# pkzhou/PointSLOT

Hardware: AMD Instinct MI355X
Metric: tracked frames/sec KITTI stereo 1242x375 (higher is better)
Workload: dtype u8

## Files before the change

### pointslot_amd/csrc/orb_plan.h

```cpp
#pragma once
#include <stdint.h>

#define PS_ORB_MAX_LEVELS 8
#define PS_EDGE 19
#define PS_MINB 16
#define PS_QT_NCAP 2048
#define PS_FAST_WIN 66

struct OrbLevel {
  int32_t w, h;
  int32_t stride;
  int32_t bstride;
  uint32_t plane_off;
  uint32_t blur_off;
  int32_t n_cols, n_rows;
  int32_t w_cell, h_cell;
  int32_t cell_base;
  int32_t cell_cap;
  uint32_t cand_off;
  uint32_t key_off;
  int32_t key_cap;
  int32_t quota;
  int32_t n_ini;
  float h_x;
  int32_t sel_off;
  int32_t sel_cap;
  float scale;
  float inv_scale;
  float kp_size;
  uint32_t xtab_off, ytab_off;
  int32_t blur_blk_base;
  int32_t border_blk_base;
};

struct OrbPlan {
  OrbLevel lv[PS_ORB_MAX_LEVELS];
  int32_t nlevels;
  int32_t img_w, img_h;
  int32_t n_cells;
  int32_t sel_total;
  int32_t kp_cap;
  int32_t ini_th, min_th;
  int32_t blur_blocks;
  int32_t border_blocks;
  uint64_t arena_bytes;
  uint64_t cellcnt_off;
  uint64_t cand_base;
  uint64_t key_base;
  uint64_t sel_base;
  uint64_t selcnt_off;
  uint64_t ncand_off;
  uint32_t celltab_off;
};

struct StPair {
  const uint8_t* arena_l; const uint8_t* arena_r;
  const void* kps_l; const uint8_t* desc_l; const int32_t* cnt_l;
  const void* kps_r; const uint8_t* desc_r; const int32_t* cnt_r;
  float* u_right; float* depth; int32_t* sad; int32_t* kept;
  uint8_t* scratch;
};
#define PS_ST_MAXB 512
#define PS_ST_CAP 4096
#define PS_ST_OFF_BYTES ((PS_ST_MAXB + 4) * 4)
#define PS_ST_SCRATCH (PS_ST_OFF_BYTES + PS_ST_CAP * 4 + PS_ST_CAP * 8)
```

### pointslot_amd/csrc/orb_stereo.hip

```cpp
#include <hip/hip_runtime.h>
#include <stdint.h>
#include "orb_plan.h"

namespace {

#define ST_G(T) const __attribute__((address_space(1))) T
#define ST_GM(T) __attribute__((address_space(1))) T
template <typename T> __device__ __forceinline__ ST_G(T)* st_g(const T* p) { return (ST_G(T)*)p; }
template <typename T> __device__ __forceinline__ ST_GM(T)* st_gm(T* p) { return (ST_GM(T)*)p; }

typedef uint32_t st_u4 __attribute__((ext_vector_type(4)));
typedef uint32_t st_u2 __attribute__((ext_vector_type(2)));
struct PsKeyPoint { float x, y, size, angle, response; int32_t octave, class_id; };

__device__ __forceinline__ int hamming256(const st_u4 a0, const st_u4 a1, const st_u4 b0, const st_u4 b1) {
  return __popc(a0.x ^ b0.x) + __popc(a0.y ^ b0.y) + __popc(a0.z ^ b0.z) + __popc(a0.w ^ b0.w) +
         __popc(a1.x ^ b1.x) + __popc(a1.y ^ b1.y) + __popc(a1.z ^ b1.z) + __popc(a1.w ^ b1.w);
}
__device__ __forceinline__ uint32_t wave_min_u32(uint32_t v) {
  v = min(v, (uint32_t)__builtin_amdgcn_update_dpp((int)v, (int)v, 0xB1, 0xF, 0xF, false));
  v = min(v, (uint32_t)__builtin_amdgcn_update_dpp((int)v, (int)v, 0x4E, 0xF, 0xF, false));
  v = min(v, (uint32_t)__builtin_amdgcn_update_dpp((int)v, (int)v, 0x141, 0xF, 0xF, false));
  v = min(v, (uint32_t)__builtin_amdgcn_update_dpp((int)v, (int)v, 0x140, 0xF, 0xF, false));
  const uint32_t a = (uint32_t)__builtin_amdgcn_readlane((int)v, 0), b = (uint32_t)__builtin_amdgcn_readlane((int)v, 16);
  const uint32_t c = (uint32_t)__builtin_amdgcn_readlane((int)v, 32), d = (uint32_t)__builtin_amdgcn_readlane((int)v, 48);
  return min(min(a, b), min(c, d));
}
__device__ __forceinline__ int wave_sum_i32(int v) {
  v += __builtin_amdgcn_update_dpp(0, v, 0xB1, 0xF, 0xF, true);
  v += __builtin_amdgcn_update_dpp(0, v, 0x4E, 0xF, 0xF, true);
  v += __builtin_amdgcn_update_dpp(0, v, 0x141, 0xF, 0xF, true);
  v += __builtin_amdgcn_update_dpp(0, v, 0x140, 0xF, 0xF, true);
  return __builtin_amdgcn_readlane(v, 0) + __builtin_amdgcn_readlane(v, 16) + __builtin_amdgcn_readlane(v, 32) + __builtin_amdgcn_readlane(v, 48);
}

__global__ __launch_bounds__(256) void st_bucket(OrbPlan plan, const StPair* pairs) {
  __shared__ int cnt[PS_ST_MAXB + 1], fill[PS_ST_MAXB];
  const StPair S = pairs[blockIdx.x];
  const int Nr = min(*S.cnt_r, PS_ST_CAP), tid = threadIdx.x;
  const PsKeyPoint* KR = reinterpret_cast<const PsKeyPoint*>(S.kps_r);
  int32_t* boff = reinterpret_cast<int32_t*>(S.scratch);
  int32_t* bidx = reinterpret_cast<int32_t*>(S.scratch + PS_ST_OFF_BYTES);
  uint2* rinfo = reinterpret_cast<uint2*>(S.scratch + PS_ST_OFF_BYTES + PS_ST_CAP * 4);
  const int nb = min(PS_ST_MAXB, (plan.img_h >> 3) + 1);
  for (int b = tid; b <= PS_ST_MAXB; b += 256) { cnt[b] = 0; if (b < PS_ST_MAXB) fill[b] = 0; }
  __syncthreads();
  for (int iR = tid; iR < Nr; iR += 256) {
    const PsKeyPoint kr = KR[iR];
    const float r = __fmul_rn(2.0f, plan.lv[kr.octave].scale);
    const int maxr = (int)ceilf(__fadd_rn(kr.y, r)), minr = (int)floorf(__fsub_rn(kr.y, r));
    (void)maxr; (void)minr;
    atomicAdd(&cnt[min(max((int)kr.y >> 3, 0), nb - 1)], 1);
  }
  __syncthreads();
  if (tid == 0) { int acc = 0; for (int b = 0; b <= nb; b++) { const int c = cnt[b]; cnt[b] = acc; acc += c; } }
  __syncthreads();
  for (int b = tid; b <= nb; b += 256) boff[b] = cnt[b];
  for (int iR = tid; iR < Nr; iR += 256) {
    const PsKeyPoint kr = KR[iR];
    const int b = min(max((int)kr.y >> 3, 0), nb - 1);
    const int pos = cnt[b] + atomicAdd(&fill[b], 1);
    const float r = __fmul_rn(2.0f, plan.lv[kr.octave].scale);
    const int maxr = (int)ceilf(__fadd_rn(kr.y, r)), minr = (int)floorf(__fsub_rn(kr.y, r));
    bidx[pos] = iR;
    rinfo[pos] = make_uint2(__float_as_uint(kr.x), (uint32_t)(min(max(minr + 1024, 0), 8191)) | ((uint32_t)(min(max(maxr + 1024, 0), 8191)) << 13) | ((uint32_t)kr.octave << 26));
  }
}

typedef unsigned short st_us2 __attribute__((ext_vector_type(2)));
__device__ __forceinline__ uint32_t row_min_u32(uint32_t v) {
  v = min(v, (uint32_t)__builtin_amdgcn_update_dpp((int)v, (int)v, 0xB1, 0xF, 0xF, false));
  v = min(v, (uint32_t)__builtin_amdgcn_update_dpp((int)v, (int)v, 0x4E, 0xF, 0xF, false));
  v = min(v, (uint32_t)__builtin_amdgcn_update_dpp((int)v, (int)v, 0x141, 0xF, 0xF, false));
  v = min(v, (uint32_t)__builtin_amdgcn_update_dpp((int)v, (int)v, 0x140, 0xF, 0xF, false));
  return v;
}
__device__ __forceinline__ int row_sum_i32(int v) {
  v += __builtin_amdgcn_update_dpp(0, v, 0xB1, 0xF, 0xF, true);
  v += __builtin_amdgcn_update_dpp(0, v, 0x4E, 0xF, 0xF, true);
  v += __builtin_amdgcn_update_dpp(0, v, 0x141, 0xF, 0xF, true);
  v += __builtin_amdgcn_update_dpp(0, v, 0x140, 0xF, 0xF, true);
  return v;
}
#define ST_PAIR(hi, lo, b0, b1) __builtin_amdgcn_perm(hi, lo, (uint32_t)(b0) | 0x0c000c00u | ((uint32_t)(b1) << 16))

__global__ __launch_bounds__(256) void st_match(OrbPlan plan, const StPair* pairs, float mb, float mbf, int npairs) {
  __shared__ float s_scale[PS_ORB_MAX_LEVELS], s_inv[PS_ORB_MAX_LEVELS];
  __shared__ int s_w[PS_ORB_MAX_LEVELS], s_stride[PS_ORB_MAX_LEVELS];
  __shared__ uint32_t s_plane[PS_ORB_MAX_LEVELS];
#pragma unroll
  for (int l = 0; l < PS_ORB_MAX_LEVELS; l++)
    if ((int)threadIdx.x == l) { s_scale[l] = plan.lv[l].scale; s_inv[l] = plan.lv[l].inv_scale; s_w[l] = plan.lv[l].w; s_stride[l] = plan.lv[l].stride; s_plane[l] = plan.lv[l].plane_off; }
  __syncthreads();
  const int pair = (int)blockIdx.y * 8 + ((int)blockIdx.x & 7);
  if (pair >= npairs) return;
  const StPair S = pairs[pair];
  const int wave = __builtin_amdgcn_readfirstlane(threadIdx.x >> 6), lane = threadIdx.x & 63, grp = lane >> 4, l16 = lane & 15;
  const int N = *st_g(S.cnt_l);
  const int iL0 = ((int)blockIdx.x >> 3) * 16 + wave * 4;
  if (iL0 >= N) return;
  const int iL = iL0 + grp;
  const bool live = iL < N;
  ST_G(PsKeyPoint)* KL = st_g(reinterpret_cast<const PsKeyPoint*>(S.kps_l));
  const int iLc = live ? iL : N - 1;
  PsKeyPoint kpL;
  kpL.x = KL[iLc].x; kpL.y = KL[iLc].y; kpL.octave = KL[iLc].octave;
  float out_ur = -1.0f, out_depth = -1.0f;
  int out_sad = -1;
  const float minD = 0.f, maxD = __fdiv_rn(mbf, mb);
  const float uL = kpL.x, vL = kpL.y;
  const int levelL = kpL.octave;
  const int rowL = (int)vL;
  const float minU = __fsub_rn(uL, maxD), maxU = __fsub_rn(uL, minD);
  uint32_t best = 0xFFFFFFFFu;
  float best_rx = 0.f;
  if (live && !(maxU < 0)) {
    ST_G(st_u4)* dl = st_g(reinterpret_cast<const st_u4*>(S.desc_l + (size_t)iL * 32));
    const st_u4 a0 = dl[0], a1 = dl[1];
    ST_G(int32_t)* boff = st_g(reinterpret_cast<const int32_t*>(S.scratch));
    ST_G(int32_t)* bidx = st_g(reinterpret_cast<const int32_t*>(S.scratch + PS_ST_OFF_BYTES));
    ST_G(st_u2)* rinfo = st_g(reinterpret_cast<const st_u2*>(S.scratch + PS_ST_OFF_BYTES + PS_ST_CAP * 4));
    const int nb = min(PS_ST_MAXB, (plan.img_h >> 3) + 1);
    const float rmax = __fadd_rn(__fmul_rn(2.0f, plan.lv[plan.nlevels - 1].scale), 2.0f);
    const int b0 = min(max((int)floorf((float)rowL - rmax) >> 3, 0), nb - 1), b1 = min(max((int)ceilf((float)rowL + rmax) >> 3, 0), nb - 1);
    const int k_end = boff[b1 + 1];
    const uint32_t rowk = (uint32_t)(rowL + 1024);
    for (int k = boff[b0] + l16; k < k_end; k += 64) {
      st_u2 ri[4]; int iR[4];
#pragma unroll
      for (int u = 0; u < 4; u++) { const int ku = min(k + 16 * u, k_end - 1); ri[u] = rinfo[ku]; iR[u] = bidx[ku]; }
#pragma unroll
      for (int u = 0; u < 4; u++) {
        if (k + 16 * u >= k_end) continue;
        const uint32_t minr = ri[u].y & 0x1FFF, maxr = (ri[u].y >> 13) & 0x1FFF;
        const int oct = (int)(ri[u].y >> 26);
        if (rowk < minr || rowk > maxr) continue;
        if ((uint32_t)(oct - levelL + 1) > 2u) continue;
        const float rx = __uint_as_float(ri[u].x);
        if (!(rx >= minU && rx <= maxU)) continue;
        ST_G(st_u4)* dr = st_g(reinterpret_cast<const st_u4*>(S.desc_r + (size_t)iR[u] * 32));
        const uint32_t d = (uint32_t)hamming256(a0, a1, dr[0], dr[1]);
        if (d < 100u) {
          const uint32_t key = (d << 16) | (uint32_t)iR[u];
          if (key < best) { best = key; best_rx = rx; }
        }
      }
    }
  }
  const uint32_t lane_best = best;
  best = row_min_u32(best);
  float uR0 = 0.f;
  {
    const uint32_t owners = (uint32_t)(__ballot(lane_best == best && best != 0xFFFFFFFFu) >> (lane & 48)) & 0xFFFFu;
    uR0 = __shfl(best_rx, (lane & 48) + (owners ? __ffs((int)owners) - 1 : 0));
  }
  const int bestDist = best == 0xFFFFFFFFu ? 100 : (int)(best >> 16);
  if (bestDist < 75) {
    const float Lscale = s_scale[levelL], Linv = s_inv[levelL];
    const int Lw = s_w[levelL], Lstride = s_stride[levelL];
    const uint32_t Lplane = s_plane[levelL];
    const float scaleduL = roundf(__fmul_rn(kpL.x, Linv));
    const float scaledvL = roundf(__fmul_rn(kpL.y, Linv));
    const float scaleduR0 = roundf(__fmul_rn(uR0, Linv));
    const float iniu = scaleduR0 + 5 - 5, endu = scaleduR0 + 5 + 5 + 1;
    if (!(iniu < 0 || endu >= (float)Lw)) {
      const int cy = (int)scaledvL, cxl = (int)scaleduL, cxr = (int)scaleduR0;
      const int i = min(l16, 10);
      ST_G(uint8_t)* al = st_g(S.arena_l);
      ST_G(uint8_t)* ar = st_g(S.arena_r);
      ST_G(uint32_t)* pl = (ST_G(uint32_t)*)(al + (Lplane + (uint32_t)((PS_EDGE + cy + i - 5) * Lstride + PS_EDGE + cxl - 5)));
      ST_G(uint32_t)* pr = (ST_G(uint32_t)*)(ar + (Lplane + (uint32_t)((PS_EDGE + cy + i - 5) * Lstride + PS_EDGE + cxr - 10)));
      ST_G(uint32_t)* prc = (ST_G(uint32_t)*)(ar + (Lplane + (uint32_t)((PS_EDGE + cy) * Lstride + PS_EDGE + cxr - 10)));
      uint32_t lw[3], rw[6], cw[6];
#pragma unroll
      for (int q = 0; q < 3; q++) lw[q] = pl[q];
#pragma unroll
      for (int q = 0; q < 6; q++) { rw[q] = pr[q]; cw[q] = prc[q]; }
      const uint32_t Lc = al[Lplane + (uint32_t)((PS_EDGE + cy) * Lstride + PS_EDGE + cxl)];
      const uint32_t biasA = (256u - Lc) * 0x00010001u;
      uint32_t a[6];
#pragma unroll
      for (int q = 0; q < 5; q++) a[q] = ST_PAIR(lw[q >> 1], lw[q >> 1], (2 * q) & 3, (2 * q + 1) & 3) + biasA;
      a[5] = ST_PAIR(0u, lw[2], 2, 0x0c) + (biasA & 0xFFFFu);
      uint32_t E[11], O[10];
#pragma unroll
      for (int q = 0; q < 11; q++) {
        const int b0i = 2 * q, b1i = 2 * q + 1;
        E[q] = ST_PAIR(rw[b0i >> 2], rw[b0i >> 2], b0i & 3, q == 10 ? 0x0c : (b1i & 3));
      }
#pragma unroll
      for (int q = 0; q < 10; q++) {
        const int b0i = 2 * q + 1, b1i = 2 * q + 2;
        O[q] = ST_PAIR(rw[b1i >> 2], rw[b0i >> 2], b0i & 3, (b1i & 3) + ((b1i >> 2) != (b0i >> 2) ? 4 : 0));
      }
      int dists[11];
#pragma unroll
      for (int s = 0; s < 11; s++) {
        const uint32_t Rc = (cw[(s + 5) >> 2] >> (8 * ((s + 5) & 3))) & 0xFFu;
        const uint32_t biasB = (256u - Rc) * 0x00010001u;
        uint32_t acc = 0;
#pragma unroll
        for (int q = 0; q < 5; q++) {
          const uint32_t r2 = (s & 1) ? O[(s - 1) / 2 + q] : E[s / 2 + q];
          acc = __builtin_amdgcn_sad_u16(a[q], r2 + biasB, acc);
        }
        const uint32_t rl = ((s & 1) ? O[(s - 1) / 2 + 5] : E[s / 2 + 5]) & 0xFFFFu;
        acc = __builtin_amdgcn_sad_u16(a[5], rl + (biasB & 0xFFFFu), acc);
        dists[s] = row_sum_i32(l16 < 11 ? (int)acc : 0);
      }
      int bestS = 0x7fffffff, bestinc = 0;
#pragma unroll
      for (int s = 0; s < 11; s++)
        if (dists[s] < bestS) { bestS = dists[s]; bestinc = s - 5; }
      if (bestinc != -5 && bestinc != 5) {
        float d1 = 0, d2 = 0, d3 = 0;
#pragma unroll
        for (int s = 1; s < 10; s++)
          if (s - 5 == bestinc) { d1 = (float)dists[s - 1]; d2 = (float)dists[s]; d3 = (float)dists[s + 1]; }
        const float deltaR = __fdiv_rn(__fsub_rn(d1, d3), __fmul_rn(2.0f, __fsub_rn(__fadd_rn(d1, d3), __fmul_rn(2.0f, d2))));
        if (!(deltaR < -1 || deltaR > 1)) {
          float bestuR = __fmul_rn(Lscale, __fadd_rn(__fadd_rn(scaleduR0, (float)bestinc), deltaR));
          float disparity = __fsub_rn(uL, bestuR);
          if (disparity >= minD && disparity < maxD) {
            if (disparity <= 0) {
              disparity = 0.01f;
              bestuR = (float)((double)uL - 0.01);
            }
            out_depth = __fdiv_rn(mbf, disparity);
            out_ur = bestuR;
            out_sad = bestS;
          }
        }
      }
    }
  }
  if (l16 == 0 && live) { st_gm(S.u_right)[iL] = out_ur; st_gm(S.depth)[iL] = out_depth; st_gm(S.sad)[iL] = out_sad; }
}

#ifndef ST_MED_T
#define ST_MED_T 256
#endif
__global__ __launch_bounds__(ST_MED_T) void st_median(OrbPlan plan, const StPair* pairs) {
  __shared__ __attribute__((aligned(16))) uint32_t keys[PS_ST_CAP + 4];
  __shared__ int nkeys, median_sad;
  __shared__ int red[ST_MED_T / 64];
  const StPair S = pairs[blockIdx.x];
  const int N = min(*S.cnt_l, PS_ST_CAP), tid = threadIdx.x;
  if (tid == 0) { nkeys = 0; median_sad = -1; }
  __syncthreads();
  for (int i = tid; i < N; i += ST_MED_T) {
    const int sd = S.sad[i];
    if (sd >= 0) keys[atomicAdd(&nkeys, 1)] = ((uint32_t)sd << 12) | (uint32_t)i;
  }
  __syncthreads();
  const int n = nkeys;
  if (n == 0) { if (tid == 0) *S.kept = 0; return; }
  if (tid < 4) keys[n + tid] = 0xFFFFFFFFu;
  __syncthreads();
  {
    __shared__ int hist[256];
    __shared__ int sel_bin, sel_rank;
    int want = n / 2;
    for (int level = 0; level < 2; level++) {
      if (tid < 256) hist[tid] = 0;
      __syncthreads();
      const int hi_bin = level == 1 ? sel_bin : 0;
      for (int e = tid; e < n; e += ST_MED_T) {
        const uint32_t sd = keys[e] >> 12;
        if (level == 0) atomicAdd(&hist[sd >> 8], 1);
        else if ((int)(sd >> 8) == hi_bin) atomicAdd(&hist[sd & 255u], 1);
      }
      __syncthreads();
      if (tid == 0) {
        int acc = 0, b = 0;
        for (; b < 256; b++) { if (acc + hist[b] > want) break; acc += hist[b]; }
        if (level == 0) { sel_bin = b; sel_rank = want - acc; }
        else median_sad = (hi_bin << 8) | b;
      }
      __syncthreads();
      want = sel_rank;
    }
  }
  const float thDist = __fmul_rn(__fmul_rn(1.5f, 1.4f), (float)median_sad);
  int kept = 0;
  for (int e = tid; e < n; e += ST_MED_T) {
    const uint32_t k = keys[e];
    const int i = (int)(k & 0xFFF);
    if ((float)(int)(k >> 12) < thDist) kept++;
    else { S.u_right[i] = -1.0f; S.depth[i] = -1.0f; }
  }
  kept = wave_sum_i32(kept);
  if ((tid & 63) == 0) red[tid >> 6] = kept;
  __syncthreads();
  if (tid == 0) { int acc = 0; for (int w = 0; w < ST_MED_T / 64; w++) acc += red[w]; *S.kept = acc; }
}

}

extern "C" void psk_stereo_launch(const OrbPlan* plan, const StPair* d_pairs, int npairs, int max_left, float mb, float mbf, hipStream_t st) {
  hipLaunchKernelGGL(st_bucket, dim3(npairs), dim3(256), 0, st, *plan, d_pairs);
  hipLaunchKernelGGL(st_match, dim3(((max_left + 15) / 16) * 8, (npairs + 7) / 8), dim3(256), 0, st, *plan, d_pairs, mb, mbf, npairs);
  hipLaunchKernelGGL(st_median, dim3(npairs), dim3(ST_MED_T), 0, st, *plan, d_pairs);
}
```

Measured before the change: 51930.

## Bucket right keypoints by octave and row, compact candidates into per-row queues

Right keypoints are now bucketed by (octave, row band) rather than row band alone, so each left keypoint scans only the three adjacent-octave ranges. Surviving candidates are compacted through a shared-memory queue per 16-lane group, so descriptor loads and Hamming distances run on full groups of lanes instead of on scattered, divergent lanes. The bucket prefix sum also becomes a parallel wave scan instead of a single-thread loop. The cost is a larger offset table, extra LDS use and wavefront barriers, plus index arithmetic to map across the three segments.

Result: faster. 52700 (median of 6 runs) (+1.5%).

```diff
diff --git a/pointslot_amd/csrc/orb_plan.h b/pointslot_amd/csrc/orb_plan.h
--- a/pointslot_amd/csrc/orb_plan.h
+++ b/pointslot_amd/csrc/orb_plan.h
@@ -62,5 +62,5 @@
 };
 #define PS_ST_MAXB 512
 #define PS_ST_CAP 4096
-#define PS_ST_OFF_BYTES ((PS_ST_MAXB + 4) * 4)
+#define PS_ST_OFF_BYTES ((PS_ORB_MAX_LEVELS * PS_ST_MAXB + 4) * 4)
 #define PS_ST_SCRATCH (PS_ST_OFF_BYTES + PS_ST_CAP * 4 + PS_ST_CAP * 8)
diff --git a/pointslot_amd/csrc/orb_stereo.hip b/pointslot_amd/csrc/orb_stereo.hip
--- a/pointslot_amd/csrc/orb_stereo.hip
+++ b/pointslot_amd/csrc/orb_stereo.hip
@@ -34,32 +34,38 @@
   return __builtin_amdgcn_readlane(v, 0) + __builtin_amdgcn_readlane(v, 16) + __builtin_amdgcn_readlane(v, 32) + __builtin_amdgcn_readlane(v, 48);
 }
 
+#define ST_NBINS (PS_ORB_MAX_LEVELS * PS_ST_MAXB)
+__device__ __forceinline__ int st_bin(const OrbPlan& plan, int nb, int octave, float y) {
+  return min(max(octave, 0), plan.nlevels - 1) * nb + min(max((int)y >> 3, 0), nb - 1);
+}
 __global__ __launch_bounds__(256) void st_bucket(OrbPlan plan, const StPair* pairs) {
-  __shared__ int cnt[PS_ST_MAXB + 1], fill[PS_ST_MAXB];
+  __shared__ int cnt[ST_NBINS + 1], wsum[4];
   const StPair S = pairs[blockIdx.x];
   const int Nr = min(*S.cnt_r, PS_ST_CAP), tid = threadIdx.x;
   const PsKeyPoint* KR = reinterpret_cast<const PsKeyPoint*>(S.kps_r);
   int32_t* boff = reinterpret_cast<int32_t*>(S.scratch);
   int32_t* bidx = reinterpret_cast<int32_t*>(S.scratch + PS_ST_OFF_BYTES);
   uint2* rinfo = reinterpret_cast<uint2*>(S.scratch + PS_ST_OFF_BYTES + PS_ST_CAP * 4);
-  const int nb = min(PS_ST_MAXB, (plan.img_h >> 3) + 1);
-  for (int b = tid; b <= PS_ST_MAXB; b += 256) { cnt[b] = 0; if (b < PS_ST_MAXB) fill[b] = 0; }
+  const int nb = min(PS_ST_MAXB, (plan.img_h >> 3) + 1), nbins = min(plan.nlevels, PS_ORB_MAX_LEVELS) * nb;
+  for (int b = tid; b <= nbins; b += 256) cnt[b] = 0;
+  __syncthreads();
+  for (int iR = tid; iR < Nr; iR += 256) atomicAdd(&cnt[st_bin(plan, nb, KR[iR].octave, KR[iR].y)], 1);
+  __syncthreads();
+  const int per = (nbins + 256) / 256, e0 = min(tid * per, nbins + 1), e1 = min(e0 + per, nbins + 1);
+  int run = 0;
+  for (int b = e0; b < e1; b++) run += cnt[b];
+  int incl = run;
+#pragma unroll
+  for (int d = 1; d < 64; d <<= 1) { const int o = __shfl_up(incl, d); if ((tid & 63) >= d) incl += o; }
+  if ((tid & 63) == 63) wsum[tid >> 6] = incl;
+  __syncthreads();
+  int acc = incl - run;
+  for (int w = 0; w < (tid >> 6); w++) acc += wsum[w];
+  for (int b = e0; b < e1; b++) { const int c = cnt[b]; cnt[b] = acc; boff[b] = acc; acc += c; }
   __syncthreads();
   for (int iR = tid; iR < Nr; iR += 256) {
     const PsKeyPoint kr = KR[iR];
-    const float r = __fmul_rn(2.0f, plan.lv[kr.octave].scale);
-    const int maxr = (int)ceilf(__fadd_rn(kr.y, r)), minr = (int)floorf(__fsub_rn(kr.y, r));
-    (void)maxr; (void)minr;
-    atomicAdd(&cnt[min(max((int)kr.y >> 3, 0), nb - 1)], 1);
-  }
-  __syncthreads();
-  if (tid == 0) { int acc = 0; for (int b = 0; b <= nb; b++) { const int c = cnt[b]; cnt[b] = acc; acc += c; } }
-  __syncthreads();
-  for (int b = tid; b <= nb; b += 256) boff[b] = cnt[b];
-  for (int iR = tid; iR < Nr; iR += 256) {
-    const PsKeyPoint kr = KR[iR];
-    const int b = min(max((int)kr.y >> 3, 0), nb - 1);
-    const int pos = cnt[b] + atomicAdd(&fill[b], 1);
+    const int pos = atomicAdd(&cnt[st_bin(plan, nb, kr.octave, kr.y)], 1);
     const float r = __fmul_rn(2.0f, plan.lv[kr.octave].scale);
     const int maxr = (int)ceilf(__fadd_rn(kr.y, r)), minr = (int)floorf(__fsub_rn(kr.y, r));
     bidx[pos] = iR;
@@ -83,11 +89,14 @@
   return v;
 }
 #define ST_PAIR(hi, lo, b0, b1) __builtin_amdgcn_perm(hi, lo, (uint32_t)(b0) | 0x0c000c00u | ((uint32_t)(b1) << 16))
+#define ST_QUEUE 80
+#define ST_ROW_SYNC() do { __builtin_amdgcn_fence(__ATOMIC_ACQ_REL, "wavefront"); __builtin_amdgcn_wave_barrier(); } while (0)
 
 __global__ __launch_bounds__(256) void st_match(OrbPlan plan, const StPair* pairs, float mb, float mbf, int npairs) {
   __shared__ float s_scale[PS_ORB_MAX_LEVELS], s_inv[PS_ORB_MAX_LEVELS];
   __shared__ int s_w[PS_ORB_MAX_LEVELS], s_stride[PS_ORB_MAX_LEVELS];
   __shared__ uint32_t s_plane[PS_ORB_MAX_LEVELS];
+  __shared__ uint2 s_queue[16][ST_QUEUE];
 #pragma unroll
   for (int l = 0; l < PS_ORB_MAX_LEVELS; l++)
     if ((int)threadIdx.x == l) { s_scale[l] = plan.lv[l].scale; s_inv[l] = plan.lv[l].inv_scale; s_w[l] = plan.lv[l].w; s_stride[l] = plan.lv[l].stride; s_plane[l] = plan.lv[l].plane_off; }
@@ -121,30 +130,65 @@
     ST_G(int32_t)* bidx = st_g(reinterpret_cast<const int32_t*>(S.scratch + PS_ST_OFF_BYTES));
     ST_G(st_u2)* rinfo = st_g(reinterpret_cast<const st_u2*>(S.scratch + PS_ST_OFF_BYTES + PS_ST_CAP * 4));
     const int nb = min(PS_ST_MAXB, (plan.img_h >> 3) + 1);
-    const float rmax = __fadd_rn(__fmul_rn(2.0f, plan.lv[plan.nlevels - 1].scale), 2.0f);
-    const int b0 = min(max((int)floorf((float)rowL - rmax) >> 3, 0), nb - 1), b1 = min(max((int)ceilf((float)rowL + rmax) >> 3, 0), nb - 1);
-    const int k_end = boff[b1 + 1];
+    int rs[3], rl[3];
+#pragma unroll
+    for (int j = 0; j < 3; j++) {
+      const int o = levelL - 1 + j;
+      rs[j] = 0; rl[j] = 0;
+      if (o >= 0 && o < plan.nlevels) {
+        const float ro = __fadd_rn(__fmul_rn(2.0f, s_scale[o]), 2.0f);
+        const int b0 = min(max((int)floorf((float)rowL - ro) >> 3, 0), nb - 1), b1 = min(max((int)ceilf((float)rowL + ro) >> 3, 0), nb - 1);
+        rs[j] = *(ST_G(int32_t)*)((ST_G(uint8_t)*)boff + ((uint32_t)(o * nb + b0) << 2));
+        rl[j] = *(ST_G(int32_t)*)((ST_G(uint8_t)*)boff + ((uint32_t)(o * nb + b1 + 1) << 2)) - rs[j];
+      }
+    }
+    const int c1 = rl[0], c2 = rl[0] + rl[1], T = c2 + rl[2];
+    const int base0 = rs[0], base1 = rs[1] - c1, base2 = rs[2] - c2;
     const uint32_t rowk = (uint32_t)(rowL + 1024);
-    for (int k = boff[b0] + l16; k < k_end; k += 64) {
+    uint2* q = s_queue[wave * 4 + grp];
+    int nq = 0;
+    for (int p0 = 0; p0 < T; p0 += 64) {
       st_u2 ri[4]; int iR[4];
 #pragma unroll
-      for (int u = 0; u < 4; u++) { const int ku = min(k + 16 * u, k_end - 1); ri[u] = rinfo[ku]; iR[u] = bidx[ku]; }
-#pragma unroll
       for (int u = 0; u < 4; u++) {
-        if (k + 16 * u >= k_end) continue;
+        const int p = min(p0 + 16 * u + l16, T - 1);
+        const uint32_t k = (uint32_t)(p + (p < c1 ? base0 : (p < c2 ? base1 : base2)));
+        ri[u] = *(ST_G(st_u2)*)((ST_G(uint8_t)*)rinfo + (k << 3)); iR[u] = *(ST_G(int32_t)*)((ST_G(uint8_t)*)bidx + (k << 2));
+      }
+#pragma unroll
+      for (int u = 0; u < 4; u++) asm volatile("" : "+v"(iR[u]), "+v"(ri[u].x), "+v"(ri[u].y));
+#pragma unroll
+      for (int u = 0; u < 4; u++) {
         const uint32_t minr = ri[u].y & 0x1FFF, maxr = (ri[u].y >> 13) & 0x1FFF;
-        const int oct = (int)(ri[u].y >> 26);
-        if (rowk < minr || rowk > maxr) continue;
-        if ((uint32_t)(oct - levelL + 1) > 2u) continue;
         const float rx = __uint_as_float(ri[u].x);
-        if (!(rx >= minU && rx <= maxU)) continue;
-        ST_G(st_u4)* dr = st_g(reinterpret_cast<const st_u4*>(S.desc_r + (size_t)iR[u] * 32));
-        const uint32_t d = (uint32_t)hamming256(a0, a1, dr[0], dr[1]);
-        if (d < 100u) {
-          const uint32_t key = (d << 16) | (uint32_t)iR[u];
-          if (key < best) { best = key; best_rx = rx; }
+        const bool pass = p0 + 16 * u + l16 < T && rowk >= minr && rowk <= maxr && rx >= minU && rx <= maxU;
+        const uint32_t rowbits = (uint32_t)(__builtin_amdgcn_ballot_w64(pass) >> (lane & 48)) & 0xFFFFu;
+        if (pass) q[nq + __popc(rowbits & ((1u << l16) - 1u))] = make_uint2((uint32_t)iR[u], ri[u].x);
+        nq += __popc(rowbits);
+      }
+      ST_ROW_SYNC();
+      const bool last = p0 + 64 >= T;
+      int head = 0;
+      while (nq >= 16 || (last && nq > 0)) {
+        const int n = min(nq, 16);
+        if (l16 < n) {
+          const uint2 c = q[head + l16];
+          ST_G(st_u4)* dr = st_g(reinterpret_cast<const st_u4*>(S.desc_r + (size_t)c.x * 32));
+          const uint32_t d = (uint32_t)hamming256(a0, a1, dr[0], dr[1]);
+          if (d < 100u) {
+            const uint32_t key = (d << 16) | c.x;
+            if (key < best) { best = key; best_rx = __uint_as_float(c.y); }
+          }
         }
-      }
+        head += 16; nq -= n;
+      }
+      if (head > 0 && nq > 0) {
+        uint2 c = make_uint2(0u, 0u);
+        if (l16 < nq) c = q[head + l16];
+        ST_ROW_SYNC();
+        if (l16 < nq) q[l16] = c;
+      }
+      ST_ROW_SYNC();
     }
   }
   const uint32_t lane_best = best;
```
